# ekzhu/datasketch

Measured on AMD Instinct MI355X. Metric: MinHash signatures/sec (1M sets x 256 tokens, num_perm=128), higher is better.
Workload: dtype u64

## Files before the change

datasketch_amd/csrc/mhx_internal.h:

```cpp
#pragma once

#include <hip/hip_runtime.h>

#include <algorithm>
#include <cstdarg>
#include <cstdint>
#include <cstdio>
#include <mutex>
#include <string>
#include <unordered_map>

#include "mhx.h"

namespace mhx {

void set_error(const char *fmt, ...);
int fail(int code, const char *fmt, ...);
void forgive();

#define MHX_HIP_CHECK(expr)                                                                      \
    do {                                                                                         \
        hipError_t _e = (expr);                                                                  \
        if (_e != hipSuccess) {                                                                  \
            return ::mhx::fail(_e == hipErrorOutOfMemory ? MHX_ERR_OOM : MHX_ERR_HIP,            \
// ... 1 lines not shown
                               __LINE__);                                                        \
        }                                                                                        \
    } while (0)

constexpr int kSigDigests = 2;
constexpr int kSigDigestsBM = 3;

constexpr unsigned int kPairListCap = 16384;
constexpr size_t kWorkBytes = 64 + sizeof(unsigned int) * kPairListCap;

#define MHX_GUARD(ctxp) std::lock_guard<std::recursive_mutex> _mhx_guard((ctxp)->mu)

#define MHX_REQUIRE(cond, ...)                                       \
    do {                                                             \
        if (!(cond)) return ::mhx::fail(MHX_ERR_INVALID, __VA_ARGS__); \
    } while (0)

hipError_t dev_malloc(void **p, size_t bytes, bool caller = false);
hipError_t dev_free(void *p);
bool guard_mode();

}

struct mhx_ctx {
    std::recursive_mutex mu;
    int device = 0;
    hipStream_t stream = nullptr;
    int num_cus = 0;
    int hw_cus = 0;
    int64_t lds_per_block = 64 << 10;
    int64_t hbm_bytes = 0;
    char name[128] = {0};
    void *scratch[5] = {nullptr, nullptr, nullptr, nullptr, nullptr};
    size_t scratch_bytes[5] = {0, 0, 0, 0, 0};
    int64_t opt_minhash_path = 0;
    int64_t opt_minhash_packed = 0;
    int64_t opt_minhash_adapt = 0;
    int64_t opt_minhash_share = 0;
    int64_t opt_minhash_p3 = 0;
    int64_t opt_minhash_ties = 0;
    int64_t opt_minhash_split = 0;
    int64_t opt_blocks_per_cu = 0;
    int64_t opt_debug_cus = 0;
    int64_t opt_minhash_prefetch = 1;
    int64_t opt_minhash_alias = -1;
    int64_t opt_weighted_path = 0;
    int64_t opt_weighted_min_dim = 0;
    int64_t opt_weighted_rescue = 0;
    int64_t opt_weighted_plan = 0;
    int64_t opt_weighted_kernel = 0;
    int64_t opt_weighted_debug = 0;
    int64_t opt_weighted_split = 0;
    int64_t opt_weighted_tail = 0;
    int64_t opt_weighted_direct = 0;
    int64_t opt_lsh_sort = 0;
    int64_t opt_lsh_gather = 0;
    int64_t opt_lsh_sort_bits = 0;
    int64_t opt_lsh_prehash = 0;
    int64_t opt_lsh_chunk = 0;
    int64_t opt_lsh_bigbins = 0;
    int64_t opt_lsh_team = 0;
    int64_t opt_lsh_merge_items = 0;
    int64_t opt_lsh_levels = 0;
    int64_t opt_pack_fused = 0;
    int64_t opt_weighted_refill = 0;
    int64_t opt_hll_split_tokens = 0;
    int64_t opt_bloom_lanes = 0;
    int64_t opt_jaccard_topk_path = 0;
    int64_t opt_jaccard_topk_segments = 0;
    int64_t opt_overlap_bins = 0;
    int64_t opt_host_chunk_bytes = 0;

    hipStream_t copy_in = nullptr;
    hipStream_t copy_out = nullptr;
    int ensure_copy_streams();

    unsigned long long *d_stats = nullptr;
    uint8_t *d_redo = nullptr;
    int64_t redo_capacity = 0;
    int64_t redo_sets = 0;
    int ensure_redo(int64_t n_sets);
    unsigned int *d_work = nullptr;
    int ensure_work();

    int ensure_scratch(int slot, size_t bytes);
    int activate() const;
};

struct mhx_perm {
    mhx_ctx *ctx = nullptr;
    int32_t num_perm = 0;
    uint64_t *d_a = nullptr;
    uint64_t *d_b = nullptr;
};

struct mhx_wgen {
    mhx_ctx *ctx = nullptr;
    int32_t sample_size = 0;
    int32_t dim = 0;
    float *d_params = nullptr;
    int32_t s_pad = 0;
    bool table_fast = false;
    float *d_aos = nullptr;
    float *d_walk_a = nullptr;
    uint32_t *d_walk_c = nullptr;
    void *d_walk_plan = nullptr;
    int plan_index = 0;
    bool walk_ok = false;
};

struct mhx_event {
    mhx_ctx *ctx = nullptr;
    hipEvent_t ev = nullptr;
};

namespace mhx {

int launch_minhash_bulk(mhx_perm *perm, const void *d_hv, int hv_dtype, const int64_t *d_offsets,
                        int64_t fixed_len, int64_t n_sets, int64_t total_tokens,
                        const uint64_t *d_init, int64_t init_stride, void *d_out, int out_dtype,
                        int64_t first_token = 0);
int launch_sha1_tokens(mhx_ctx *ctx, const uint8_t *d_bytes, const int64_t *d_offsets, int64_t n_tokens,
                       int out_dtype, void *d_out);
int launch_sha1_windows(mhx_ctx *ctx, const uint8_t *d_bytes, const int64_t *d_item_offsets, const int64_t *d_doc_offsets,
                        const int64_t *d_set_offsets, int64_t n_docs, int64_t n_windows, int64_t width, int out_dtype, void *d_out);
int launch_words_count(mhx_ctx *ctx, const uint8_t *d_bytes, int64_t n_bytes, const int64_t *d_doc_offsets, int64_t n_docs,
                       const uint8_t *table, int64_t *n_words, int64_t *n_out_bytes);
int launch_words_emit(mhx_ctx *ctx, const uint8_t *d_bytes, int64_t n_bytes, const int64_t *d_doc_offsets, int64_t n_docs,
                      const uint8_t *table, uint8_t *d_out, int64_t *d_item_offsets, int64_t *d_word_doc_offsets);
int launch_minhash_merge(mhx_ctx *ctx, const uint64_t *d_x, const uint64_t *d_y, int64_t count,
                         uint64_t *d_out);
int launch_weighted(mhx_wgen *gen, const int64_t *d_indptr, const int32_t *d_indices,
                    const float *d_values, int values_are_logs, int64_t n_rows, int64_t nnz,
                    int64_t *d_out, uint8_t *d_nonempty);
int launch_weighted_log(mhx_ctx *ctx, const float *d_x, int64_t n, float *d_out);
int launch_wgen_transpose(mhx_wgen *gen, const float *d_rs, const float *d_lncs, const float *d_betas);
int launch_bbit_pack(mhx_ctx *ctx, const void *d_sig, int sig_dtype, int64_t n, int32_t k, int32_t b,
                     uint64_t *d_out);
int launch_band_keys(mhx_ctx *ctx, const uint64_t *d_sig, int64_t n, int32_t k, int32_t bands,
                     int32_t r, uint64_t *d_out);
int launch_band_digests(mhx_ctx *ctx, const void *d_sig, int sig_dtype, int64_t n, int32_t k, int32_t bands, int32_t r,
                        uint64_t *d_out, int layout = 0);
int launch_bbit_digest_fused(mhx_ctx *ctx, const void *d_sig, int sig_dtype, int64_t n, int32_t k, int32_t b, int32_t bands,
                             int32_t r, uint64_t *d_blocks, uint64_t *d_digests, int layout, bool *done);
int launch_jaccard_pairs(mhx_ctx *ctx, const void *d_a, const void *d_b, int sig_dtype, int32_t k, const int64_t *d_pairs,
                         int64_t m, int32_t *d_counts);
int launch_weighted_dense(mhx_wgen *gen, const float *d_x, int values_are_logs, int64_t n_rows, int64_t *d_out,
                          uint8_t *d_nonempty);
int launch_lsh_candidate_pairs(mhx_ctx *ctx, const uint64_t *d_sorted_digests, const uint32_t *d_sorted_rows, int64_t n,
                               int32_t bands, int64_t *d_pairs, int64_t capacity, int64_t *n_pairs, int64_t *n_raw);
int launch_lsh_sort_bands(mhx_ctx *ctx, const void *d_sig, int sig_dtype, int64_t n, int32_t k, int32_t bands, int32_t r,
                          uint64_t *d_sorted_digests, uint32_t *d_sorted_rows);
int launch_lsh_query(mhx_ctx *ctx, const uint64_t *d_sorted_digests, const uint32_t *d_sorted_rows, int64_t n, int32_t bands,
                     int32_t r, const void *d_q_sig, const void *d_idx_sig, int sig_dtype, int32_t k, int64_t m,
                     int64_t *d_pairs, int64_t capacity, int64_t *n_pairs);
int launch_lsh_ensemble_query(mhx_ctx *ctx, const mhx_ensemble_level *levels, int32_t n_levels, const int64_t *start, int32_t n_parts,
                              const void *d_idx_sig, int sig_dtype, int32_t k, const void *d_q_sig, int64_t m, const uint8_t *d_choice,
                              const int32_t *params, int32_t n_params, int64_t *d_pairs, int64_t capacity, int64_t *n_pairs);
int launch_bbit_jaccard(mhx_ctx *ctx, const uint64_t *d_a, const uint64_t *d_b, int32_t k, int32_t b, const int64_t *d_pairs,
                        int64_t m, int32_t *d_counts);
int launch_lean_serialize(mhx_ctx *ctx, const void *d_sig, int sig_dtype, int64_t n, int32_t k, int64_t seed, int big_endian,
                          uint8_t *d_out);
int launch_lean_deserialize(mhx_ctx *ctx, const uint8_t *d_records, int64_t n, int32_t k, int big_endian, int sig_dtype, void *d_sig,
                            int64_t *d_seeds, unsigned int *d_bad);
int launch_bbit_unpack(mhx_ctx *ctx, const uint64_t *d_blocks, int64_t n, int32_t k, int32_t b, uint32_t *d_out);

// ... 60 lines not shown
```

datasketch_amd/csrc/minhash_kernels.hip:

```cpp
#include <type_traits>

#include "mhx_internal.h"

namespace mhx {
namespace {

constexpr uint64_t kMersenne = (1ull << 61) - 1;
constexpr uint32_t kMaxHash = 0xFFFFFFFFu;
constexpr int kWave = 64;

struct BulkArgs {
    const void *hv;
    const int64_t *offsets;
    int64_t fixed_len;
    int64_t n_sets;
    const uint64_t *a;
    const uint64_t *b;
    int32_t num_perm;
    int32_t path;
    unsigned long long *stats;
    uint8_t *redo;
    int32_t redo_match;
    unsigned int *sieve_hint;
    unsigned int *mode_word;
    unsigned int *pair_count;
    unsigned int *pair_list;
    int32_t prefetch;
    int32_t ties;
    int32_t share_last;
    int64_t alias_mask;
    const uint64_t *init;
    int64_t init_stride;
    void *out;
};

__device__ __forceinline__ void mad_narrow(uint32_t h, uint32_t a_lo, uint32_t a_hi, uint64_t b,
                                           uint32_t &s_lo, uint32_t &s_hi) {
    const uint64_t s0 = (uint64_t)h * a_lo + b;
    s_lo = (uint32_t)s0;
    s_hi = (uint32_t)(s0 >> 32) + h * a_hi;
}

__device__ __forceinline__ void mad_wide(uint32_t h_lo, uint32_t h_hi, uint32_t a_lo, uint32_t a_hi,
                                         uint64_t b, uint32_t &s_lo, uint32_t &s_hi) {
    const uint64_t s0 = (uint64_t)h_lo * a_lo + b;
    s_lo = (uint32_t)s0;
    s_hi = (uint32_t)(s0 >> 32) + h_lo * a_hi + h_hi * a_lo;
}

__device__ __forceinline__ uint32_t fold_exact(uint32_t s_lo, uint32_t s_hi) {
    const uint32_t top = s_hi >> 29;
    const uint64_t y = ((((uint64_t)(s_hi & 0x1FFFFFFFu)) << 32) | s_lo) + top;
    return (uint32_t)y + (y >= kMersenne ? 1u : 0u);
}

__device__ __forceinline__ uint32_t fold_fast(uint32_t s_lo, uint32_t s_hi) {
    return s_lo + (s_hi >> 29);
}

template <bool EXACT>
__device__ __forceinline__ uint32_t fold(uint32_t s_lo, uint32_t s_hi) {
    return EXACT ? fold_exact(s_lo, s_hi) : fold_fast(s_lo, s_hi);
}

template <int P>
struct Perms {
    uint32_t a_lo[P], a_hi[P];
    uint64_t b[P];
};

#define MHX_CONST_AS __attribute__((address_space(4)))
template <typename T>
__device__ __forceinline__ const T MHX_CONST_AS *as_const(const T *p) {
    return (const T MHX_CONST_AS *)p;
}

template <typename TokT>
struct Chunk;
template <>
struct Chunk<uint64_t> {
    static constexpr int N = 8;
    uint32_t w[2 * N];
    __device__ __forceinline__ void load(const uint64_t MHX_CONST_AS *p) {
        const uint32_t MHX_CONST_AS *q = (const uint32_t MHX_CONST_AS *)p;
#pragma unroll
        for (int i = 0; i < 2 * N; ++i) w[i] = q[i];
    }
    __device__ __forceinline__ uint32_t or_hi() const {
        uint32_t o = 0;
#pragma unroll
        for (int i = 0; i < N; ++i) o |= w[2 * i + 1];
        return o;
    }
    __device__ __forceinline__ uint32_t lo(int i) const { return w[2 * i]; }
    __device__ __forceinline__ uint32_t hi(int i) const { return w[2 * i + 1]; }
    __device__ __forceinline__ void keep_whole() const {
        asm volatile("" ::"s"(w[1]), "s"(w[3]), "s"(w[5]), "s"(w[7]), "s"(w[9]), "s"(w[11]), "s"(w[13]), "s"(w[15]));
    }
    __device__ __forceinline__ void arrived() const { asm volatile("" ::"s"(w[0])); }
};
template <>
struct Chunk<uint32_t> {
    static constexpr int N = 16;
    uint32_t v[N];
    __device__ __forceinline__ void load(const uint32_t MHX_CONST_AS *p) {
#pragma unroll
        for (int i = 0; i < N; ++i) v[i] = p[i];
    }
    __device__ __forceinline__ uint32_t or_hi() const { return 0; }
    __device__ __forceinline__ uint32_t lo(int i) const { return v[i]; }
    __device__ __forceinline__ uint32_t hi(int) const { return 0; }
    __device__ __forceinline__ void keep_whole() const {}
// ... 595 lines not shown
    int gap = 16;
    int streak = 0;
    __device__ __forceinline__ void failed() {
        if (++streak >= 2) {
            skip = gap;
            gap = min(2 * gap, 64);
        }
    }
    __device__ __forceinline__ void succeeded() {
        streak = 0;
        gap = 16;
    }
};

struct TiesBackoff {
    int skip = 0;
    int score = 0;
    __device__ __forceinline__ void failed() {
        score += 4;
        if (score >= 8) {
            skip = 32;
            score = 4;
        }
    }
    __device__ __forceinline__ void succeeded() { score = max(score - 1, 0); }
};

template <int P, typename TokT>
__device__ __forceinline__ void set_minima(const BulkArgs &args, const TokT MHX_CONST_AS *hv, const TokT *hv_vec,
                                           int64_t beg, int64_t end, const Perms<P> &pm,
                                           const Perms<P> &pm_biased, const SievePerms<P> &sp, int kbase,
                                           int lane, uint32_t *lds, SieveBackoff &bo, uint32_t (&res)[P]) {
    bool full = args.path != 0;
    if (!full) {
        if (bo.skip > 0) {
            --bo.skip;
            full = true;
        } else {
            full = sieve_minima<P, TokT>(hv, hv_vec, beg, end, pm, pm_biased, sp, args.stats, lane, lds, res);
            if (full) {
                if (args.stats && lane == 0) atomicAdd(args.stats, 1ull);
                bo.failed();
            } else {
                bo.succeeded();
            }
        }
    }
    if (full) {
        const Minima<P> m = full_minima<P, TokT>(hv_vec, beg, end, args.a, args.b, args.num_perm, kbase,
                                                 args.path == 1, args.stats);
#pragma unroll
        for (int p = 0; p < P; ++p) res[p] = m.v[p];
    }
}

template <int P, bool SHARE = false>
__device__ __forceinline__ void load_perms(const BulkArgs &args, int kbase, int lane, Perms<P> &pm,
                                           Perms<P> &pm_biased, SievePerms<P> &sp, int (&kidx)[P]) {
    uint32_t span = kWave;
    if constexpr (SHARE && P >= 3) {
        const int r = args.num_perm - (kbase + (P - 1) * kWave);
        span = r > 16 ? 32u : r > 8 ? 16u : r > 4 ? 8u : 4u;
    }
    sp.span = span;
#pragma unroll
    for (int p = 0; p < P; ++p) {
        const bool shared = SHARE && P >= 3 && p == P - 1;
        const int k = kbase + p * kWave + (shared ? lane & (int)(span - 1) : lane);
        const bool holds = k < args.num_perm;
        kidx[p] = holds && !(shared && lane >= (int)span) ? k : -1;
        const uint64_t a = holds ? args.a[k] : 0;
        pm.a_lo[p] = (uint32_t)a;
        pm.a_hi[p] = (uint32_t)(a >> 32);
        pm.b[p] = holds ? args.b[k] : 0;
        pm_biased.a_lo[p] = pm.a_lo[p];
        pm_biased.a_hi[p] = pm.a_hi[p];
        pm_biased.b[p] = pm.b[p] + 1;
        sp.a_lo[p] = pm.a_lo[p];
        sp.b8[p] = pm.b[p] + 8;
        sp.active[p] = kidx[p] >= 0;
    }
}

enum { MODE_SIEVE = 0, MODE_FULL = 1, MODE_DEDUP = 2, MODE_SIEVE_TIES = 3 };
enum { SHAPE_GENERAL = 0, SHAPE_PLAIN = 1, SHAPE_PLAIN_FIXED = 2, SHAPE_PLAIN_FIXED_ROWS = 3 };

template <int P, typename TokT, typename OutT, int MODE, int SHAPE, bool SHARE = false>
__global__ __launch_bounds__(256) void minhash_bulk_kernel(const BulkArgs args_in) {
    BulkArgs args = args_in;
    constexpr bool kSieve = MODE == MODE_SIEVE || MODE == MODE_SIEVE_TIES;
    if (kSieve && args.mode_word) {
        const unsigned int want_ties = *as_const(args.mode_word);
        if ((want_ties == 1u) != (MODE == MODE_SIEVE_TIES)) return;
    }
    if (MODE == MODE_FULL && args.mode_word && args.sieve_hint && blockIdx.x == 0 && threadIdx.x == 0) {
        const unsigned int t = __builtin_nontemporal_load(args.sieve_hint), f = __builtin_nontemporal_load(args.sieve_hint + 1);
        const unsigned int g = __builtin_nontemporal_load(args.sieve_hint + 2), m = *args.mode_word;
        const unsigned int tt = __builtin_nontemporal_load(args.sieve_hint + 3), tf = __builtin_nontemporal_load(args.sieve_hint + 5);
        if (t >= 64u) {
            const bool defeated = 4u * f > t;
            const bool heavy = m == 1u ? 5u * g > t : (tt >= 64u ? 5u * tf > tt : m == 2u);
            *args.mode_word = !defeated ? 0u : heavy ? 2u : 1u;
        }
    }
    if (SHAPE != SHAPE_GENERAL) {
        args.init = nullptr;
        args.init_stride = 0;
        args.stats = nullptr;
        args.alias_mask = -1;
    }
    if (SHAPE == SHAPE_PLAIN_FIXED || SHAPE == SHAPE_PLAIN_FIXED_ROWS) args.offsets = nullptr;
    const int lane = threadIdx.x & (kWave - 1);
    const int wave = __builtin_amdgcn_readfirstlane(threadIdx.x >> 6);
    const int waves_per_block = blockDim.x >> 6;
    const int kchunks = (args.num_perm + kWave * P - 1) / (kWave * P);
    constexpr int kLdsPerWave = MODE == MODE_DEDUP ? kDedupWordsPerWave : kStageWordsPerWave;
    __shared__ __attribute__((aligned(16))) uint32_t stage[4 * kLdsPerWave];
    uint32_t *lds = stage + wave * kLdsPerWave;
    Perms<P> pm, pm_biased;
    SievePerms<P> sp;
    int kidx[P];
    if (kSieve || MODE == MODE_DEDUP) load_perms<P, SHARE>(args, 0, lane, pm, pm_biased, sp, kidx);

    const TokT MHX_CONST_AS *hv = as_const(static_cast<const TokT *>(args.hv));
    const TokT *hv_vec = static_cast<const TokT *>(args.hv);
    const int64_t MHX_CONST_AS *offsets = as_const(args.offsets);
    OutT *__restrict__ out = static_cast<OutT *>(args.out);
    const int64_t stride = (int64_t)gridDim.x * waves_per_block;
    const bool flagged_only = !kSieve && args.redo != nullptr;
    unsigned int listed_n = 0;
    bool listed = false;
    if (MODE == MODE_FULL && flagged_only && args.pair_list) {
        listed_n = *as_const(args.pair_count);
        listed = listed_n <= kPairListCap;
    }
    const int64_t n_items = listed ? (int64_t)listed_n : flagged_only ? (args.n_sets + kWave - 1) / kWave * waves_per_block : args.n_sets;
    SieveBackoff backoff;
    TiesBackoff ties;
    int tried = 0, failed = 0, left = 0;
    if (MODE == MODE_SIEVE && args.sieve_hint) {
        const unsigned int t = __builtin_nontemporal_load(args.sieve_hint), f = __builtin_nontemporal_load(args.sieve_hint + 1);
        if (t >= 64u && 2u * f > t) {
            backoff.skip = 63;
            backoff.gap = 64;
            backoff.streak = 2;
        }
    }
    if (MODE == MODE_FULL && listed) {
        uint32_t *comb = stage;
        for (int64_t it = blockIdx.x; it < (int64_t)listed_n; it += gridDim.x) {
            const int64_t set = (int64_t)as_const(args.pair_list)[it];
            const int64_t beg = args.offsets ? offsets[set] : set * args.fixed_len;
            const int64_t end = args.offsets ? offsets[set + 1] : beg + args.fixed_len;
            const int64_t share = (end - beg + 31) / 32 * 8;
            const int64_t wbeg = min(end, beg + wave * share), wend = min(end, wbeg + share);
            for (int kc = 0; kc < kchunks; ++kc) {
                uint32_t mine[P];
#pragma unroll
                for (int p = 0; p < P; ++p) mine[p] = kMaxHash;
                if (wend > wbeg) {
                    const Minima<P> m = full_minima<P, TokT>(hv_vec, wbeg, wend, args.a, args.b, args.num_perm, kc * (kWave * P),
                                                             args.path == 1, args.stats);
#pragma unroll
                    for (int p = 0; p < P; ++p) mine[p] = m.v[p];
                }
#pragma unroll
                for (int p = 0; p < P; ++p) comb[(wave * P + p) * kWave + lane] = mine[p];
                __syncthreads();
                if (wave == 0) {
#pragma unroll
                    for (int p = 0; p < P; ++p) {
                        const int k = kc * (kWave * P) + p * kWave + lane;
                        if (k >= args.num_perm) continue;
                        uint32_t r = mine[p];
#pragma unroll
                        for (int w = 1; w < 4; ++w) r = min(r, comb[(w * P + p) * kWave + lane]);
                        uint64_t v = r;
                        if (args.init) {
                            const uint64_t iv = args.init[set * args.init_stride + k];
                            v = end > beg ? (uint64_t)min((iv >> 32) ? kMaxHash : (uint32_t)iv, r) : iv;
                        }
                        if (sizeof(OutT) == 4) v = v > kMaxHash ? kMaxHash : v;
                        out[set * args.num_perm + k] = (OutT)v;
                    }
                }
                __syncthreads();
            }
        }
        return;
    }
    for (int64_t item0 = (int64_t)blockIdx.x * waves_per_block + wave; item0 < n_items; item0 += stride) {
      const int64_t item = flagged_only ? item0 / waves_per_block : item0;
      unsigned long long todo = 1;
      if (flagged_only && !listed) {
          const int64_t cand = item * kWave + lane;
          const bool mine = (lane % waves_per_block) == (int)(item0 % waves_per_block);
          todo = __ballot(mine && cand < args.n_sets && args.redo[cand] == (uint8_t)args.redo_match);
      }
      while (todo) {
        const int bit = __builtin_ctzll(todo);
        todo &= todo - 1;
        const int64_t set = listed ? (int64_t)as_const(args.pair_list)[item0] : flagged_only ? item * kWave + bit : item;
        int64_t beg, end;
        if (args.offsets) {
            beg = offsets[set];
            end = offsets[set + 1];
        } else {
            beg = (args.alias_mask >= 0 ? (set & args.alias_mask) : set) * args.fixed_len;
            end = beg + args.fixed_len;
        }
        uint32_t warm = 0;
        {
            const int64_t nset = listed ? args.n_sets : flagged_only ? (todo ? item * kWave + __builtin_ctzll(todo) : args.n_sets) : item + stride;
            const bool skipping_on = MODE == MODE_SIEVE && backoff.skip > 1;
            if (args.prefetch && nset < args.n_sets && !skipping_on) {
                const int64_t nbeg = args.offsets ? offsets[nset] : nset * args.fixed_len;
                const int64_t nend = args.offsets ? offsets[nset + 1] : nbeg + args.fixed_len;
                const int64_t off = (int64_t)lane * 128;
                if (off < (nend - nbeg) * (int64_t)sizeof(TokT))
                    warm = *reinterpret_cast<const volatile uint32_t *>(reinterpret_cast<const char *>(args.hv) +
                                                                         nbeg * (int64_t)sizeof(TokT) + off);
            }
        }
        bool defer = false;
        if (MODE == MODE_SIEVE && end > beg && backoff.skip > 0) {
            --backoff.skip;
            defer = true;
        }
        for (int kc = 0; kc < kchunks && !defer; ++kc) {
            uint32_t res[P];
            if (kSieve) {
                if (kchunks > 1) load_perms<P, SHARE>(args, kc * (kWave * P), lane, pm, pm_biased, sp, kidx);
                if (end > beg) {
                    bool tied = false;
                    defer = sieve_minima<P, TokT, SHAPE != SHAPE_PLAIN_FIXED_ROWS, MODE == MODE_SIEVE_TIES, SHARE>(hv, hv_vec, beg, end, pm, pm_biased, sp, args.stats, lane, lds, res,
                                                                                                          MODE == MODE_SIEVE_TIES ? &tied : nullptr);
                    if (kc == 0) ++tried;
                    if (MODE == MODE_SIEVE_TIES) {
                        if (defer || __any(tied)) ++failed;
                        if (defer) {
                            ++left;
                            break;
                        }
                    } else {
                        if (defer) {
                            ++failed;
                            backoff.failed();
                            break;
                        }
                        backoff.succeeded();
                    }
                }
            } else {
#pragma unroll
                for (int p = 0; p < P; ++p) {
                    const int k = kc * (kWave * P) + p * kWave + lane;
                    kidx[p] = k < args.num_perm ? k : -1;
                }
                if (end > beg) {
                    if (MODE == MODE_DEDUP) {
                        if (kchunks > 1) load_perms<P>(args, kc * (kWave * P), lane, pm, pm_biased, sp, kidx);
                        bool open = true;
                        if (!args.ties || (args.mode_word && *as_const(args.mode_word) == 1u)) {
                        } else if (ties.skip > 0) {
                            if (kc == kchunks - 1) --ties.skip;
                        } else {
                            open = sieve_minima<P, TokT, true, true>(hv, hv_vec, beg, end, pm, pm_biased, sp, nullptr, lane, lds, res);
                            if (kc == 0) ++tried, failed += open ? 1 : 0;
                            if (open) ties.failed(); else ties.succeeded();
                        }
                        if (open) {
#pragma unroll
                        for (int p = 0; p < P; ++p) res[p] = kMaxHash;
                        uint64_t cur[4];
                        load_quad<TokT>(hv_vec, beg, end, lane, cur);
                        defer = __any(dedup_sieve_range<P, TokT>(hv_vec, beg, end, pm, sp, lds, lane, cur, res));
                        if (defer) {
                            if (args.stats && lane == 0) atomicAdd(args.stats + 3, 1ull);
                            break;
                        }
                        }
                    } else {
                        const Minima<P> m = full_minima<P, TokT>(hv_vec, beg, end, args.a, args.b, args.num_perm,
                                                                 kc * (kWave * P), args.path == 1, args.stats);
#pragma unroll
                        for (int p = 0; p < P; ++p) res[p] = m.v[p];
                    }
                }
            }
#pragma unroll
            for (int p = 0; p < P; ++p) {
                if (kidx[p] < 0) continue;
                uint64_t v;
                if (args.init) {
                    const uint64_t iv = args.init[set * args.init_stride + kidx[p]];
                    if (end > beg) {
                        const uint32_t ic = (iv >> 32) ? kMaxHash : (uint32_t)iv;
                        v = min(ic, res[p]);
                    } else {
                        v = iv;
                    }
                } else {
                    v = end > beg ? res[p] : kMaxHash;
                }
                if (sizeof(OutT) == 4) v = v > kMaxHash ? kMaxHash : v;
// ... 180 lines not shown
    const int wave = __builtin_amdgcn_readfirstlane(threadIdx.x >> 6);
    const int waves_per_block = blockDim.x >> 6;
    __shared__ __attribute__((aligned(16))) uint32_t stage[4 * kStageWordsPerWave];
    uint32_t *lds = stage + wave * kStageWordsPerWave;
    Perms<P> pm, pm_biased;
    SievePerms<P> sp;
    int kidx[P];
    load_perms<P>(args, blockIdx.y * (kWave * P), lane, pm, pm_biased, sp, kidx);
    const TokT MHX_CONST_AS *hv = as_const(static_cast<const TokT *>(args.hv));
    const TokT *hv_vec = static_cast<const TokT *>(args.hv);
    const int64_t MHX_CONST_AS *offsets = as_const(args.offsets);
    OutT *__restrict__ out = static_cast<OutT *>(args.out);

    const int64_t n_slices = (total_tokens + slice - 1) / slice;
    const int64_t stride = (int64_t)gridDim.x * waves_per_block;
    SieveBackoff backoff;
    for (int64_t s = (int64_t)blockIdx.x * waves_per_block + wave; s < n_slices; s += stride) {
        const int64_t s_beg = first_token + s * slice;
        const int64_t s_end = min(s_beg + slice, first_token + total_tokens);
        int64_t set;
        if (args.offsets) {
            int64_t lo = 0, hi = args.n_sets;
            while (hi - lo > 1) {
                const int64_t mid = (lo + hi) >> 1;
                if (offsets[mid] <= s_beg) lo = mid; else hi = mid;
            }
            set = lo;
        } else {
            set = s_beg / args.fixed_len;
        }
        for (; set < args.n_sets; ++set) {
            const int64_t set_beg = args.offsets ? offsets[set] : set * args.fixed_len;
            const int64_t set_end = args.offsets ? offsets[set + 1] : set_beg + args.fixed_len;
            if (set_beg >= s_end) break;
            const int64_t beg = max(set_beg, s_beg), end = min(set_end, s_end);
            if (end <= beg) continue;
            uint32_t res[P];
            set_minima<P, TokT>(args, hv, hv_vec, beg, end, pm, pm_biased, sp, blockIdx.y * (kWave * P), lane, lds, backoff, res);
#pragma unroll
            for (int p = 0; p < P; ++p) {
                if (kidx[p] < 0) continue;
                OutT *dst = out + set * args.num_perm + kidx[p];
                if (sizeof(OutT) == 8)
                    atomicMin(reinterpret_cast<unsigned long long *>(dst), (unsigned long long)res[p]);
                else
                    atomicMin(reinterpret_cast<unsigned int *>(dst), res[p]);
            }
        }
    }
}

__global__ void minhash_merge_kernel(const uint64_t *__restrict__ x, const uint64_t *__restrict__ y,
                                     int64_t count, uint64_t *__restrict__ out) {
    const int64_t n2 = count >> 1;
    const ulonglong2 *x2 = reinterpret_cast<const ulonglong2 *>(x);
    const ulonglong2 *y2 = reinterpret_cast<const ulonglong2 *>(y);
    ulonglong2 *o2 = reinterpret_cast<ulonglong2 *>(out);
    const int64_t stride = (int64_t)gridDim.x * blockDim.x;
    for (int64_t i = (int64_t)blockIdx.x * blockDim.x + threadIdx.x; i < n2; i += 4 * stride) {
        ulonglong2 xa[4], ya[4];
#pragma unroll
        for (int u = 0; u < 4; ++u) {
            if (i + u * stride < n2) {
                xa[u].x = __builtin_nontemporal_load(&x2[i + u * stride].x);
                xa[u].y = __builtin_nontemporal_load(&x2[i + u * stride].y);
                ya[u].x = __builtin_nontemporal_load(&y2[i + u * stride].x);
                ya[u].y = __builtin_nontemporal_load(&y2[i + u * stride].y);
            }
        }
#pragma unroll
        for (int u = 0; u < 4; ++u) {
            if (i + u * stride >= n2) break;
            ulonglong2 r;
            r.x = xa[u].x < ya[u].x ? xa[u].x : ya[u].x;
            r.y = xa[u].y < ya[u].y ? xa[u].y : ya[u].y;
            __builtin_nontemporal_store(r.x, &o2[i + u * stride].x);
            __builtin_nontemporal_store(r.y, &o2[i + u * stride].y);
        }
    }
    if ((count & 1) && blockIdx.x == 0 && threadIdx.x == 0)
        out[count - 1] = x[count - 1] < y[count - 1] ? x[count - 1] : y[count - 1];
}

unsigned resident_grid(mhx_ctx *ctx, const void *kernel, int64_t items) {
    int per_cu = 0;
    if (hipOccupancyMaxActiveBlocksPerMultiprocessor(&per_cu, kernel, 256, 0) != hipSuccess || per_cu < 1) {
        (void)hipGetLastError();
        per_cu = 2;
    }
    return (unsigned)std::max<int64_t>(1, std::min<int64_t>(items, (int64_t)ctx->num_cus * per_cu));
}

template <int P, typename TokT, typename OutT, int PF = P>
int launch_typed(mhx_ctx *ctx, const BulkArgs &args, int64_t first_token, int64_t total_tokens, bool split) {
    const int kchunks = (args.num_perm + kWave * P - 1) / (kWave * P);
    const int blocks_per_cu = ctx->opt_blocks_per_cu > 0 ? (int)ctx->opt_blocks_per_cu : (P >= 3 ? 128 : 64);
    const int64_t max_blocks = (int64_t)ctx->num_cus * blocks_per_cu;
    if (!split) {
        const int64_t want = (args.n_sets + 3) / 4;
        dim3 grid((unsigned)std::max<int64_t>(1, std::min(want, max_blocks)), 1u);
        if (args.path == 0) {
            if (int rc = ctx->ensure_work()) return rc;
            MHX_HIP_CHECK(hipMemsetAsync(ctx->d_work, 0, 8 * sizeof(unsigned int), ctx->stream));
            BulkArgs sieve_args = args;
            sieve_args.sieve_hint = ctx->d_work;
            sieve_args.mode_word = ctx->opt_minhash_adapt == 1 || args.stats ? nullptr : ctx->d_work + 8;
            const BulkArgs &args_s = sieve_args;
            const bool plain = !args.init && !args.stats && args.alias_mask < 0;
            const int np = args.num_perm;
            const bool packable = !args.stats && args.alias_mask < 0 && ctx->opt_minhash_packed != 1;
            const bool packed = packable && P <= 2 && (np <= 96 || (ctx->opt_minhash_packed == 2 && np <= 128));
            if (packed) {
                const int kp = np <= 8 ? 8 : np <= 16 ? 16 : np <= 32 ? 32 : np <= 64 ? 16 : np <= 96 ? 32 : 64;
                const int64_t items = (args.n_sets + 64 / kp - 1) / (64 / kp);
                dim3 pgrid((unsigned)std::max<int64_t>(1, std::min<int64_t>((items + 3) / 4, max_blocks)), 1u);
#define MHX_PACKED(KP_, P_) hipLaunchKernelGGL((minhash_packed_kernel<KP_, P_, TokT, OutT>), pgrid, dim3(256), 0, ctx->stream, args_s)
                if (np <= 8) MHX_PACKED(8, 1);
                else if (np <= 16) MHX_PACKED(16, 1);
                else if (np <= 32) MHX_PACKED(32, 1);
                else if (np <= 48) MHX_PACKED(16, 3);
                else if (np <= 64) MHX_PACKED(16, 4);
                else if (np <= 96) MHX_PACKED(32, 3);
                else MHX_PACKED(64, 2);
#undef MHX_PACKED
            } else {
            const bool fixed_rows = plain && !args.offsets && args.fixed_len % kRowTokens == 0;
            const int last_slot = args.num_perm - (P - 1) * kWave;
            const bool share = P >= 3 && kchunks == 1 && args.share_last && last_slot > 0 && last_slot <= 32;
            const auto first_launches = [&](auto share_tag) {
                constexpr bool SH = decltype(share_tag)::value;
#define MHX_SIEVE(MODE_, SHAPE_) hipLaunchKernelGGL((minhash_bulk_kernel<P, TokT, OutT, MODE_, SHAPE_, SH>), grid, dim3(256), 0, ctx->stream, args_s)
                if (fixed_rows) MHX_SIEVE(MODE_SIEVE, SHAPE_PLAIN_FIXED_ROWS);
                else if (plain && !args.offsets) MHX_SIEVE(MODE_SIEVE, SHAPE_PLAIN_FIXED);
                else if (plain) MHX_SIEVE(MODE_SIEVE, SHAPE_PLAIN);
                else MHX_SIEVE(MODE_SIEVE, SHAPE_GENERAL);
                if (args_s.mode_word) {
                    if (fixed_rows) MHX_SIEVE(MODE_SIEVE_TIES, SHAPE_PLAIN_FIXED_ROWS);
                    else MHX_SIEVE(MODE_SIEVE_TIES, SHAPE_GENERAL);
                }
#undef MHX_SIEVE
            };
            if constexpr (P >= 3) {
                if (share) first_launches(std::true_type());
                else first_launches(std::false_type());
            } else {
                (void)share;
                first_launches(std::false_type());
            }
            }
            const int64_t flag_groups = (args.n_sets + kWave - 1) / kWave;
            BulkArgs dedup = args;
            dedup.redo_match = 1;
            dedup.sieve_hint = sieve_args.sieve_hint;
            dedup.mode_word = packed ? nullptr : sieve_args.mode_word;
            if (args.n_sets <= 0xFFFFFFFFll) {
                dedup.pair_count = ctx->d_work + 4;
                dedup.pair_list = ctx->d_work + 16;
            }
            hipLaunchKernelGGL((minhash_bulk_kernel<PF, TokT, OutT, MODE_DEDUP, SHAPE_GENERAL>),
                               dim3(resident_grid(ctx, (const void *)minhash_bulk_kernel<PF, TokT, OutT, MODE_DEDUP, SHAPE_GENERAL>, flag_groups)),
                               dim3(256), 0, ctx->stream, dedup);
            BulkArgs rest = dedup;
            rest.redo_match = 2;
            hipLaunchKernelGGL((minhash_bulk_kernel<PF, TokT, OutT, MODE_FULL, SHAPE_GENERAL>),
                               dim3(resident_grid(ctx, (const void *)minhash_bulk_kernel<PF, TokT, OutT, MODE_FULL, SHAPE_GENERAL>, flag_groups)),
                               dim3(256), 0, ctx->stream, rest);
        } else {
            BulkArgs all = args;
            all.redo = nullptr;
            hipLaunchKernelGGL((minhash_bulk_kernel<PF, TokT, OutT, MODE_FULL, SHAPE_GENERAL>), grid, dim3(256), 0, ctx->stream, all);
        }
    } else {
        const int64_t total_out = args.n_sets * (int64_t)args.num_perm;
        const int64_t fill_blocks = std::max<int64_t>(1, std::min<int64_t>((total_out + 255) / 256, max_blocks));
        hipLaunchKernelGGL((minhash_fill_state_kernel<OutT>), dim3((unsigned)fill_blocks), dim3(256), 0,
                           ctx->stream, args);
        const int64_t waves = (int64_t)ctx->num_cus * 32;
        int64_t slice = (total_tokens + waves - 1) / waves;
        slice = slice > 128 ? (slice + 255) / 256 * 256 : std::max<int64_t>(64, (slice + 15) / 16 * 16);
        const int64_t n_slices = (total_tokens + slice - 1) / slice;
        const int64_t want = (n_slices + 3) / 4;
        dim3 grid((unsigned)std::max<int64_t>(1, std::min(want, max_blocks)), (unsigned)kchunks);
        hipLaunchKernelGGL((minhash_split_kernel<P, TokT, OutT>), grid, dim3(256), 0, ctx->stream, args,
                           first_token, total_tokens, slice);
    }
    MHX_HIP_CHECK(hipGetLastError());
    return MHX_OK;
}

template <typename TokT, typename OutT>
int launch_p(mhx_ctx *ctx, const BulkArgs &args, int64_t first_token, int64_t total_tokens, bool split) {
    if (args.num_perm <= 64) return launch_typed<1, TokT, OutT>(ctx, args, first_token, total_tokens, split);
    const auto slots = [&](int p) { return (args.num_perm + kWave * p - 1) / (kWave * p) * p; };
    const bool may3 = !split && ctx->opt_minhash_p3 != 1, may4 = !split && sizeof(TokT) == 8;
    int best = 2;
    if (may3 && slots(3) <= slots(best)) best = 3;
    if (may4 && slots(4) <= slots(best)) best = 4;
    if (best == 3) return launch_typed<3, TokT, OutT, 2>(ctx, args, first_token, total_tokens, split);
    if (best == 4) return launch_typed<4, TokT, OutT, 2>(ctx, args, first_token, total_tokens, split);
    return launch_typed<2, TokT, OutT>(ctx, args, first_token, total_tokens, split);
}

}

int launch_minhash_bulk(mhx_perm *perm, const void *d_hv, int hv_dtype, const int64_t *d_offsets,
                        int64_t fixed_len, int64_t n_sets, int64_t total_tokens,
                        const uint64_t *d_init, int64_t init_stride, void *d_out, int out_dtype, int64_t first_token) {
    mhx_ctx *ctx = perm->ctx;
    if (n_sets == 0) return MHX_OK;
    total_tokens -= first_token;
    BulkArgs args;
    args.hv = d_hv;
    args.offsets = d_offsets;
    args.fixed_len = fixed_len;
    args.n_sets = n_sets;
    args.a = perm->d_a;
    args.b = perm->d_b;
    args.num_perm = perm->num_perm;
    args.path = (int32_t)ctx->opt_minhash_path;
    args.stats = ctx->d_stats;
    args.redo = nullptr;
    args.redo_match = 1;
    args.sieve_hint = nullptr;
    args.mode_word = nullptr;
    args.alias_mask = ctx->opt_minhash_alias;
    args.pair_count = nullptr;
    args.pair_list = nullptr;
    args.prefetch = ctx->opt_minhash_prefetch == 2 || (ctx->opt_minhash_prefetch == 1 && (d_offsets != nullptr || fixed_len < 256));
    args.ties = ctx->opt_minhash_ties != 1;
    args.share_last = ctx->opt_minhash_share != 1;
    args.init = d_init;
    args.init_stride = init_stride;
    args.out = d_out;
    const int64_t waves_avail = (int64_t)ctx->num_cus * 16;
    bool split = n_sets < waves_avail && total_tokens > n_sets * 128 && total_tokens >= 1024;
    if (ctx->opt_minhash_split == 1) split = false;
    if (ctx->opt_minhash_split == 2) split = total_tokens > 0;
    ctx->redo_sets = 0;
    if (!split && args.path == 0) {
        if (int rc = ctx->ensure_redo(n_sets)) return rc;
        args.redo = ctx->d_redo;
        ctx->redo_sets = n_sets;
    }
    if (hv_dtype == MHX_U64 && out_dtype == MHX_U64) return launch_p<uint64_t, uint64_t>(ctx, args, first_token, total_tokens, split);
    if (hv_dtype == MHX_U64 && out_dtype == MHX_U32) return launch_p<uint64_t, uint32_t>(ctx, args, first_token, total_tokens, split);
    if (hv_dtype == MHX_U32 && out_dtype == MHX_U64) return launch_p<uint32_t, uint64_t>(ctx, args, first_token, total_tokens, split);
    if (hv_dtype == MHX_U32 && out_dtype == MHX_U32) return launch_p<uint32_t, uint32_t>(ctx, args, first_token, total_tokens, split);
    return fail(MHX_ERR_INVALID, "unknown hv_dtype/out_dtype (%d, %d)", hv_dtype, out_dtype);
}

int launch_minhash_merge(mhx_ctx *ctx, const uint64_t *d_x, const uint64_t *d_y, int64_t count,
                         uint64_t *d_out) {
    if (count == 0) return MHX_OK;
    const int64_t want = ((count >> 1) + 1023) / 1024;
    const int64_t blocks = std::max<int64_t>(1, std::min<int64_t>(want, (int64_t)ctx->num_cus * 32));
    hipLaunchKernelGGL(minhash_merge_kernel, dim3((unsigned)blocks), dim3(256), 0, ctx->stream, d_x, d_y,
                       count, d_out);
    MHX_HIP_CHECK(hipGetLastError());
    return MHX_OK;
}

}
```

Before: 495.2 million.

## Rebalance flagged-set redo passes with striped partitioning and cached occupancy

```diff
diff --git a/datasketch_amd/csrc/mhx_internal.h b/datasketch_amd/csrc/mhx_internal.h
--- a/datasketch_amd/csrc/mhx_internal.h
+++ b/datasketch_amd/csrc/mhx_internal.h
@@ -107,6 +107,7 @@
     int ensure_redo(int64_t n_sets);
     unsigned int *d_work = nullptr;
     int ensure_work();
+    std::unordered_map<const void *, int> blocks_per_cu;
 
     int ensure_scratch(int slot, size_t bytes);
     int activate() const;
diff --git a/datasketch_amd/csrc/minhash_kernels.hip b/datasketch_amd/csrc/minhash_kernels.hip
--- a/datasketch_amd/csrc/minhash_kernels.hip
+++ b/datasketch_amd/csrc/minhash_kernels.hip
@@ -28,6 +28,7 @@
     int32_t prefetch;
     int32_t ties;
     int32_t share_last;
+    int32_t flag_parts;
     int64_t alias_mask;
     const uint64_t *init;
     int64_t init_stride;
@@ -789,6 +790,54 @@
     }
 }
 
+constexpr int kFlagStripe = 1024;
+constexpr int kFlagPartsMax = 64;
+
+__device__ __forceinline__ uint32_t flagged_share(const uint8_t *redo, int64_t n_sets, int64_t stripe, uint32_t match, uint32_t part,
+                                                  uint32_t parts, int lane) {
+    const int64_t first = stripe * kFlagStripe + lane * 16;
+    uint32_t live = 0, mine = 0;
+    if (first < n_sets) {
+        const uint4 q = *reinterpret_cast<const uint4 *>(redo + first);
+        const uint32_t w[4] = {q.x, q.y, q.z, q.w};
+#pragma unroll
+        for (int j = 0; j < 16; ++j) {
+            const uint32_t flag = (w[j >> 2] >> (8 * (j & 3))) & 0xFFu;
+            if (first + j < n_sets && flag >= match) {
+                live |= 1u << j;
+                if (flag == match) mine |= 1u << j;
+            }
+        }
+    }
+    if (__ballot(mine != 0) == 0) return 0;
+    if (parts == 1) return mine;
+    const uint32_t parts_inv = ((1u << 20) + parts - 1) / parts;
+    uint32_t before = 0, share = 0;
+#pragma unroll
+    for (int j = 0; j < 16; ++j) {
+        const unsigned long long b = __ballot((live >> j) & 1u);
+        if (b == 0) continue;
+        const uint32_t rank = before + __builtin_amdgcn_mbcnt_hi((uint32_t)(b >> 32), __builtin_amdgcn_mbcnt_lo((uint32_t)b, 0u));
+        if (rank - ((rank * parts_inv) >> 20) * parts == part) share |= mine & (1u << j);
+        before += (uint32_t)__popcll(b);
+    }
+    return share;
+}
+
+__device__ __forceinline__ int flagged_pick(uint32_t share, unsigned long long todo) {
+    const int owner = __builtin_ctzll(todo);
+    return owner * 16 + __builtin_ctz((uint32_t)__builtin_amdgcn_readlane((int)share, owner));
+}
+
+template <typename TokT>
+__device__ __forceinline__ uint32_t warm_set(const BulkArgs &args, const int64_t MHX_CONST_AS *offsets, int64_t set, int lane) {
+    const int64_t beg = args.offsets ? offsets[set] : set * args.fixed_len;
+    const int64_t end = args.offsets ? offsets[set + 1] : beg + args.fixed_len;
+    const int64_t off = (int64_t)lane * 128;
+    if (off >= (end - beg) * (int64_t)sizeof(TokT)) return 0;
+    return *reinterpret_cast<const volatile uint32_t *>(reinterpret_cast<const char *>(args.hv) + beg * (int64_t)sizeof(TokT) + off);
+}
+
 enum { MODE_SIEVE = 0, MODE_FULL = 1, MODE_DEDUP = 2, MODE_SIEVE_TIES = 3 };
 enum { SHAPE_GENERAL = 0, SHAPE_PLAIN = 1, SHAPE_PLAIN_FIXED = 2, SHAPE_PLAIN_FIXED_ROWS = 3 };
 
@@ -841,7 +890,7 @@
         listed_n = *as_const(args.pair_count);
         listed = listed_n <= kPairListCap;
     }
-    const int64_t n_items = listed ? (int64_t)listed_n : flagged_only ? (args.n_sets + kWave - 1) / kWave * waves_per_block : args.n_sets;
+    const int64_t n_items = listed ? (int64_t)listed_n : flagged_only ? (args.n_sets + kFlagStripe - 1) / kFlagStripe * args.flag_parts : args.n_sets;
     SieveBackoff backoff;
     TiesBackoff ties;
     int tried = 0, failed = 0, left = 0;
@@ -897,17 +946,29 @@
         return;
     }
     for (int64_t item0 = (int64_t)blockIdx.x * waves_per_block + wave; item0 < n_items; item0 += stride) {
-      const int64_t item = flagged_only ? item0 / waves_per_block : item0;
+      const int64_t item = flagged_only ? (int64_t)((uint32_t)item0 / (uint32_t)args.flag_parts) : item0;
       unsigned long long todo = 1;
-      if (flagged_only && !listed) {
-          const int64_t cand = item * kWave + lane;
-          const bool mine = (lane % waves_per_block) == (int)(item0 % waves_per_block);
-          todo = __ballot(mine && cand < args.n_sets && args.redo[cand] == (uint8_t)args.redo_match);
+      uint32_t share = 0;
+      bool warm_on = false;
+      if (flagged_only) {
+          int scan_lane = lane;
+          asm volatile("" : "+v"(scan_lane));
+          share = flagged_share(args.redo, args.n_sets, item, (uint32_t)args.redo_match, (uint32_t)item0 % (uint32_t)args.flag_parts,
+                                (uint32_t)args.flag_parts, scan_lane);
+          todo = __ballot(share != 0);
+          warm_on = MODE == MODE_DEDUP && (args.prefetch == 1 || (args.prefetch == 2 && __popcll(todo) <= 2));
+          if (todo && warm_on) (void)warm_set<TokT>(args, offsets, item * kFlagStripe + flagged_pick(share, todo), scan_lane);
       }
       while (todo) {
-        const int bit = __builtin_ctzll(todo);
-        todo &= todo - 1;
-        const int64_t set = listed ? (int64_t)as_const(args.pair_list)[item0] : flagged_only ? item * kWave + bit : item;
+        int64_t set = item;
+        if (flagged_only) {
+            const int owner = __builtin_ctzll(todo);
+            set = item * kFlagStripe + flagged_pick(share, todo);
+            if (lane == owner) share &= share - 1;
+            todo = __ballot(share != 0);
+        } else {
+            todo = 0;
+        }
         int64_t beg, end;
         if (args.offsets) {
             beg = offsets[set];
@@ -918,16 +979,9 @@
         }
         uint32_t warm = 0;
         {
-            const int64_t nset = listed ? args.n_sets : flagged_only ? (todo ? item * kWave + __builtin_ctzll(todo) : args.n_sets) : item + stride;
+            const int64_t nset = flagged_only ? (todo ? item * kFlagStripe + flagged_pick(share, todo) : args.n_sets) : item + stride;
             const bool skipping_on = MODE == MODE_SIEVE && backoff.skip > 1;
-            if (args.prefetch && nset < args.n_sets && !skipping_on) {
-                const int64_t nbeg = args.offsets ? offsets[nset] : nset * args.fixed_len;
-                const int64_t nend = args.offsets ? offsets[nset + 1] : nbeg + args.fixed_len;
-                const int64_t off = (int64_t)lane * 128;
-                if (off < (nend - nbeg) * (int64_t)sizeof(TokT))
-                    warm = *reinterpret_cast<const volatile uint32_t *>(reinterpret_cast<const char *>(args.hv) +
-                                                                         nbeg * (int64_t)sizeof(TokT) + off);
-            }
+            if ((flagged_only ? warm_on : args.prefetch != 0) && nset < args.n_sets && !skipping_on) warm = warm_set<TokT>(args, offsets, nset, lane);
         }
         bool defer = false;
         if (MODE == MODE_SIEVE && end > beg && backoff.skip > 0) {
@@ -1274,13 +1328,40 @@
         out[count - 1] = x[count - 1] < y[count - 1] ? x[count - 1] : y[count - 1];
 }
 
-unsigned resident_grid(mhx_ctx *ctx, const void *kernel, int64_t items) {
-    int per_cu = 0;
-    if (hipOccupancyMaxActiveBlocksPerMultiprocessor(&per_cu, kernel, 256, 0) != hipSuccess || per_cu < 1) {
-        (void)hipGetLastError();
-        per_cu = 2;
-    }
-    return (unsigned)std::max<int64_t>(1, std::min<int64_t>(items, (int64_t)ctx->num_cus * per_cu));
+int64_t resident_blocks(mhx_ctx *ctx, const void *kernel) {
+    auto it = ctx->blocks_per_cu.find(kernel);
+    if (it == ctx->blocks_per_cu.end()) {
+        int per_cu = 0;
+        if (hipOccupancyMaxActiveBlocksPerMultiprocessor(&per_cu, kernel, 256, 0) != hipSuccess || per_cu < 1) {
+            (void)hipGetLastError();
+            per_cu = 2;
+        }
+        it = ctx->blocks_per_cu.emplace(kernel, per_cu).first;
+    }
+    return (int64_t)ctx->num_cus * it->second;
+}
+
+int flag_parts(int64_t stripes, int64_t waves) {
+    int best = 1, full = 0;
+    int64_t full_trips = 0;
+    double best_busy = 0;
+    for (int parts = 1; parts <= kFlagPartsMax; ++parts) {
+        const int64_t items = stripes * parts, trips = (items + waves - 1) / waves;
+        const double busy = (double)items / (double)(trips * waves);
+        if (busy >= 0.985 && (!full || trips < full_trips)) full = parts, full_trips = trips;
+        if (busy > best_busy) best_busy = busy, best = parts;
+    }
+    return full ? full : best;
+}
+
+template <typename Kernel>
+void launch_flagged(mhx_ctx *ctx, Kernel kernel, BulkArgs args) {
+    const int64_t blocks = resident_blocks(ctx, (const void *)kernel);
+    const int64_t stripes = (args.n_sets + kFlagStripe - 1) / kFlagStripe;
+    args.flag_parts = flag_parts(stripes, blocks * 4);
+    while (args.flag_parts > 1 && stripes * args.flag_parts > 0xFFFFFFFFll) --args.flag_parts;
+    const int64_t want = (stripes * args.flag_parts + 3) / 4;
+    hipLaunchKernelGGL(kernel, dim3((unsigned)std::max<int64_t>(1, std::min(want, blocks))), dim3(256), 0, ctx->stream, args);
 }
 
 template <int P, typename TokT, typename OutT, int PF = P>
@@ -1340,23 +1421,19 @@
                 first_launches(std::false_type());
             }
             }
-            const int64_t flag_groups = (args.n_sets + kWave - 1) / kWave;
             BulkArgs dedup = args;
             dedup.redo_match = 1;
+            if (!args.prefetch && args.alias_mask < 0 && ctx->opt_minhash_prefetch != 0) dedup.prefetch = 2;
             dedup.sieve_hint = sieve_args.sieve_hint;
             dedup.mode_word = packed ? nullptr : sieve_args.mode_word;
             if (args.n_sets <= 0xFFFFFFFFll) {
                 dedup.pair_count = ctx->d_work + 4;
                 dedup.pair_list = ctx->d_work + 16;
             }
-            hipLaunchKernelGGL((minhash_bulk_kernel<PF, TokT, OutT, MODE_DEDUP, SHAPE_GENERAL>),
-                               dim3(resident_grid(ctx, (const void *)minhash_bulk_kernel<PF, TokT, OutT, MODE_DEDUP, SHAPE_GENERAL>, flag_groups)),
-                               dim3(256), 0, ctx->stream, dedup);
+            launch_flagged(ctx, minhash_bulk_kernel<PF, TokT, OutT, MODE_DEDUP, SHAPE_GENERAL>, dedup);
             BulkArgs rest = dedup;
             rest.redo_match = 2;
-            hipLaunchKernelGGL((minhash_bulk_kernel<PF, TokT, OutT, MODE_FULL, SHAPE_GENERAL>),
-                               dim3(resident_grid(ctx, (const void *)minhash_bulk_kernel<PF, TokT, OutT, MODE_FULL, SHAPE_GENERAL>, flag_groups)),
-                               dim3(256), 0, ctx->stream, rest);
+            launch_flagged(ctx, minhash_bulk_kernel<PF, TokT, OutT, MODE_FULL, SHAPE_GENERAL>, rest);
         } else {
             BulkArgs all = args;
             all.redo = nullptr;
@@ -1421,6 +1498,7 @@
     args.prefetch = ctx->opt_minhash_prefetch == 2 || (ctx->opt_minhash_prefetch == 1 && (d_offsets != nullptr || fixed_len < 256));
     args.ties = ctx->opt_minhash_ties != 1;
     args.share_last = ctx->opt_minhash_share != 1;
+    args.flag_parts = 1;
     args.init = d_init;
     args.init_stride = init_stride;
     args.out = d_out;
```

After: 497.6 million (median of 6 runs). About the same (+0.5%).
